# AaltoML/free-hunch

Measured on AMD Instinct MI355X. Metric: images/sec (256x256, num_steps=30, FH-Heun), higher is better.
Workload: dtype f32 UNet (convolutions: exact 3-way bf16 split on the bf16 MFMA, fp32 accuracy) + f64 covariance/CG; 1 GPU; FFHQ-256 arch, gaussian_blur, FH low-rank covariance (dct_diagonal), num_steps=30 heun, batch=8 per GPU; lockstep_groups_per_gpu=2, unet_backend=hip, net_calls_per_image=59

## Files before the change

### free-hunch_amd/csrc/fh_unet.hip

```cpp
#include "fh_common.h"
#include <stdlib.h>

typedef float float16_t __attribute__((ext_vector_type(16)));

namespace {

constexpr int kBK = 32;
constexpr int kLd = kBK + 4;

struct ConvArgs {
  const float* in;
  const float* w;
  const float* bias;
  const float* res;
  float* out;
  int N, H, W, Cin, Cout, KH, KW, pad, stride, Ho, Wo;
  int ksplit;
  float* ws;
};

__device__ __forceinline__ void xcd_tile(int& tile_m, int& tile_n) {
  const unsigned gx = gridDim.x, gy = gridDim.y;
  const unsigned total = gx * gy;
  unsigned lin = blockIdx.y * gx + blockIdx.x;
// ... 740 lines not shown
        if (new_row) load_a(ncc, nky);
      }
      compute(kx, c & 1);
      __syncthreads();
      if (new_row) {
        store_a();
        __syncthreads();
      }
    }
    FH_PHASE(flat_id, 2);
  } else if (!SPLIT || c_begin < c_end) {
  load_a(c_begin / 9, (c_begin / 3) % 3);
  load_b(c_begin / 9, c_begin % 9);
  store_a();
  store_b(0);
  __syncthreads();
  for (int c = c_begin; c < c_end; ++c) {
    const int kx = c % 3;
    const int nx = c + 1;
    const bool more = nx < c_end;
    const bool new_row = more && (nx % 3 == 0);
    if (more) {
      const int ncc = nx / 9, nky = (nx / 3) % 3, nkx = nx % 3;
      load_b(ncc, nky * 3 + nkx);
      if (new_row) load_a(ncc, nky);
    }
    {
      compute(kx, 0);
      __syncthreads();
      if (more) {
        store_b(0);
        if (new_row) store_a();
        __syncthreads();
      }
    }
  }
  }
  const int64_t M = (int64_t)a.N * a.Ho * a.Wo;
  const bool gn = !SPLIT && a.gn_partial != nullptr;
  float* dst = SPLIT ? a.ws + (int64_t)blockIdx.z * M * a.Cout : a.out;
  GnAcc gsum[NI];
#pragma unroll
  for (int j = 0; j < NI; ++j) {
    gsum[j].s0 = gsum[j].s1 = 0.f;
    const int co = n0 + wn + j * 32 + lr;
    if (co >= a.Cout) continue;
    const float bv = (!SPLIT && a.bias != nullptr) ? a.bias[co] : 0.f;
    float tb[5] = {0.f, 0.f, 0.f, 0.f, 0.f};
    if (gn && a.gn_mode == 1) {
#pragma unroll
      for (int q = 0; q < 5; ++q) tb[q] = a.gn_tab[((int64_t)pn * 5 + q) * a.Cout + co];
    }
    if (TT && a.wide) {
      const int k = lane & 3;
      const bool has_res = a.res != nullptr, has_x = gn && a.gn_mode == 1;
#pragma unroll
      for (int i = 0; i < MI; ++i) {
        float4 rw[4], xw[4];
        const int64_t off0 = (m0 + wm + i * 32 + 4 * lh + k) * a.Cout + (co - k);
#pragma unroll
        for (int g = 0; g < 4; ++g) {
          const int64_t off = off0 + (int64_t)(8 * g) * a.Cout;
          rw[g] = has_res ? *reinterpret_cast<const float4*>(a.res + off) : make_float4(0.f, 0.f, 0.f, 0.f);
          xw[g] = has_x ? *reinterpret_cast<const float4*>(a.gn_x + off) : make_float4(0.f, 0.f, 0.f, 0.f);
        }
#pragma unroll
        for (int g = 0; g < 4; ++g) {
          float r4[4] = {rw[g].x, rw[g].y, rw[g].z, rw[g].w}, x4[4] = {xw[g].x, xw[g].y, xw[g].z, xw[g].w}, v4[4];
          if (has_res) quad_transpose(r4, k);
          if (has_x) quad_transpose(x4, k);
#pragma unroll
          for (int q = 0; q < 4; ++q) {
            float v = acc[i][j][4 * g + q];
            v += bv;
            if (has_res) v += r4[q];
            v4[q] = v;
            if (gn) gn_accum_x(a, gsum[j], v, x4[q], tb);
          }
          quad_transpose(v4, k);
          *reinterpret_cast<float4*>(dst + off0 + (int64_t)(8 * g) * a.Cout) = make_float4(v4[0], v4[1], v4[2], v4[3]);
        }
      }
      continue;
    }
#pragma unroll
    for (int i = 0; i < MI; ++i) {
#pragma unroll
      for (int r = 0; r < 16; ++r) {
        const int64_t row = m0 + wm + i * 32 + (r & 3) + 8 * (r >> 2) + 4 * lh;
        if (row < M) {
          float v = acc[i][j][r];
          if (F16 && NP == 2) v = v * ssc.inv_in * ssc.winv;
          v += bv;
          if (!SPLIT && a.res != nullptr) v += a.res[row * a.Cout + co];
          dst[row * a.Cout + co] = v;
          if (gn) gn_accum(a, gsum[j], v, row, co, tb);
        }
      }
    }
  }
  if (GL == 1) FH_PHASE(flat_id, 3);
  if (gn) gn_reduce<NI, BM / 64, WN, BN>(a, gsum, gred, pn, (rem / BM) * (int)gridDim.y + tile_n, n0);
  if (GL == 1) FH_PHASE_EXIT(flat_id);
}

constexpr int kWK = 16;
constexpr int kWLd = kWK + 4;

template <int TB>
__global__ __launch_bounds__(512) void k_conv_wino(ConvArgs a) {
  constexpr int BN = 64;
  __shared__ __align__(16) float Ds[2][2][TB + 2][kWLd];
  __shared__ __align__(16) float Us[2][4][BN][kWLd];
  const int tid = threadIdx.x, lane = tid & 63, wave = tid >> 6;
  constexpr int MI = TB / 128;
  const int wm = (wave >> 1) * (32 * MI), wn = (wave & 1) * 32;
  const int lr = lane & 31, lh = lane >> 5;
  const int Wt = a.W / 2;
  const int64_t Mt = (int64_t)a.N * a.H * Wt;
  const int64_t t0 = (int64_t)blockIdx.x * TB;
  const int n0 = blockIdx.y * BN;
  const int cpt = a.Cin / kWK;
  const int nchunks = 3 * cpt;

  constexpr int NI = (TB + 2) * 8 / 512 + 1;
  int it_y[NI], it_slot[NI], it_q[NI];
  int64_t it_base[NI];
  bool it_ok[NI];
#pragma unroll
  for (int e = 0; e < NI; ++e) {
    const int item = tid + 512 * e;
    const bool has = e < NI - 1 || tid < 16;
    const int ps = item >> 2;
    it_q[e] = (item & 3) * 4;
    it_slot[e] = ps;
    const int64_t tg = t0 + (ps >> 1) - 1;
    it_ok[e] = has && tg >= 0 && tg < Mt;
    it_y[e] = 0;
    it_base[e] = 0;
    if (it_ok[e]) {
      const int n = (int)(tg / ((int64_t)a.H * Wt));
      const int rem = (int)(tg % ((int64_t)a.H * Wt));
      it_y[e] = rem / Wt;
      const int x = (rem % Wt) * 2 + (ps & 1);
      it_base[e] = (((int64_t)n * a.H) * a.W + x) * a.Cin + it_q[e];
    }
    if (!has) it_slot[e] = -1;
  }
  const int ub_pos[2] = {tid >> 8, 2 + (tid >> 8)};
  const int ub_co = (tid >> 2) & 63, ub_q = (tid & 3) * 4;
  const bool uvalid = n0 + ub_co < a.Cout;

  float4 rd[NI], ru[2];
  auto load_chunk = [&](int c) {
    const int ky = c / cpt, c0 = (c % cpt) * kWK;
#pragma unroll
    for (int e = 0; e < NI; ++e) {
      const int hy = it_y[e] + ky - 1;
      const bool ok = it_ok[e] && hy >= 0 && hy < a.H;
      rd[e] = ok ? *reinterpret_cast<const float4*>(a.in + it_base[e] + (int64_t)hy * a.W * a.Cin + c0)
                 : make_float4(0.f, 0.f, 0.f, 0.f);
    }
#pragma unroll
    for (int e = 0; e < 2; ++e) {
      const float* up = a.w + (((int64_t)ub_pos[e] * a.Cout + (uvalid ? n0 + ub_co : 0)) * 3 + ky) * a.Cin + c0 + ub_q;
      ru[e] = uvalid ? *reinterpret_cast<const float4*>(up) : make_float4(0.f, 0.f, 0.f, 0.f);
    }
  };
  auto store_chunk = [&](int buf) {
#pragma unroll
    for (int e = 0; e < NI; ++e)
      if (it_slot[e] >= 0) *reinterpret_cast<float4*>(&Ds[buf][it_slot[e] & 1][it_slot[e] >> 1][it_q[e]]) = rd[e];
    *reinterpret_cast<float4*>(&Us[buf][ub_pos[0]][ub_co][ub_q]) = ru[0];
    *reinterpret_cast<float4*>(&Us[buf][ub_pos[1]][ub_co][ub_q]) = ru[1];
  };

  float mfirst[MI], mlast[MI];
#pragma unroll
  for (int i = 0; i < MI; ++i) {
    const int64_t tg = t0 + wm + i * 32 + lr;
    const int xt = (int)(tg % Wt);
    mfirst[i] = xt == 0 ? 0.f : 1.f;
    mlast[i] = xt == Wt - 1 ? 0.f : 1.f;
  }

  float16_t acc[4][MI];
#pragma unroll
  for (int p = 0; p < 4; ++p)
#pragma unroll
    for (int i = 0; i < MI; ++i)
#pragma unroll
      for (int r = 0; r < 16; ++r) acc[p][i][r] = 0.f;

  load_chunk(0);
  store_chunk(0);
  __syncthreads();
  for (int c = 0; c < nchunks; ++c) {
    const int buf = c & 1;
    if (c + 1 < nchunks) load_chunk(c + 1);
#pragma unroll
    for (int g = 0; g < kWK / 8; ++g) {
      const int ko = g * 8 + 4 * lh;
      float4 v[4][MI], bf[4];
#pragma unroll
      for (int p = 0; p < 4; ++p) bf[p] = *reinterpret_cast<const float4*>(&Us[buf][p][wn + lr][ko]);
#pragma unroll
      for (int i = 0; i < MI; ++i) {
        const int sl = wm + i * 32 + lr + 1;
        const float4 d1 = *reinterpret_cast<const float4*>(&Ds[buf][0][sl][ko]);
        const float4 d2 = *reinterpret_cast<const float4*>(&Ds[buf][1][sl][ko]);
        const float4 d0 = *reinterpret_cast<const float4*>(&Ds[buf][1][sl - 1][ko]);
        const float4 d3 = *reinterpret_cast<const float4*>(&Ds[buf][0][sl + 1][ko]);
        const float f0 = mfirst[i], f3 = mlast[i];
        v[0][i] = make_float4(fmaf(d0.x, f0, -d2.x), fmaf(d0.y, f0, -d2.y), fmaf(d0.z, f0, -d2.z), fmaf(d0.w, f0, -d2.w));
        v[1][i] = make_float4(d1.x + d2.x, d1.y + d2.y, d1.z + d2.z, d1.w + d2.w);
        v[2][i] = make_float4(d2.x - d1.x, d2.y - d1.y, d2.z - d1.z, d2.w - d1.w);
        v[3][i] = make_float4(fmaf(-d3.x, f3, d1.x), fmaf(-d3.y, f3, d1.y), fmaf(-d3.z, f3, d1.z), fmaf(-d3.w, f3, d1.w));
      }
#pragma unroll
      for (int s4 = 0; s4 < 4; ++s4) {
#pragma unroll
        for (int p = 0; p < 4; ++p) {
          const float bv = s4 == 0 ? bf[p].x : s4 == 1 ? bf[p].y : s4 == 2 ? bf[p].z : bf[p].w;
#pragma unroll
          for (int i = 0; i < MI; ++i) {
            const float av = s4 == 0 ? v[p][i].x : s4 == 1 ? v[p][i].y : s4 == 2 ? v[p][i].z : v[p][i].w;
            acc[p][i] = __builtin_amdgcn_mfma_f32_32x32x2f32(av, bv, acc[p][i], 0, 0, 0);
          }
        }
      }
    }
    if (c + 1 < nchunks) store_chunk(buf ^ 1);
    __syncthreads();
  }

  const int co = n0 + wn + lr;
  if (co >= a.Cout) return;
  const float bv = a.bias != nullptr ? a.bias[co] : 0.f;
#pragma unroll
  for (int i = 0; i < MI; ++i) {
#pragma unroll
    for (int r = 0; r < 16; ++r) {
      const int64_t t = t0 + wm + i * 32 + (r & 3) + 8 * (r >> 2) + 4 * lh;
      if (t >= Mt) continue;
      const int n = (int)(t / ((int64_t)a.H * Wt));
      const int rem = (int)(t % ((int64_t)a.H * Wt));
      const int64_t pix = ((int64_t)n * a.H + rem / Wt) * a.W + (rem % Wt) * 2;
      float y0 = acc[0][i][r] + acc[1][i][r] + acc[2][i][r] + bv;
      float y1 = acc[1][i][r] - acc[2][i][r] - acc[3][i][r] + bv;
      if (a.res != nullptr) {
        y0 += a.res[pix * a.Cout + co];
        y1 += a.res[(pix + 1) * a.Cout + co];
      }
      a.out[pix * a.Cout + co] = y0;
      a.out[(pix + 1) * a.Cout + co] = y1;
    }
  }
}

template <int NO>
__global__ __launch_bounds__(256) void k_conv_thin(const float* __restrict__ in, const float* __restrict__ w,
                                                   const float* __restrict__ bias, float* __restrict__ out, int H,
                                                   int W, int Cin, int Cout) {
  constexpr int TS = 16, HS = TS + 2, LD = 36;
  __shared__ __align__(16) float xs[HS * HS][LD];
  const int tid = threadIdx.x, tx = tid & 15, ty = tid >> 4;
  const int x0 = blockIdx.x * TS, y0 = blockIdx.y * TS;
  const int64_t img = blockIdx.z;
  const float* src = in + img * H * W * Cin;
  float acc[NO];
#pragma unroll
  for (int o = 0; o < NO; ++o) acc[o] = 0.f;
  for (int c0 = 0; c0 < Cin; c0 += 32) {
    for (int idx = tid; idx < HS * HS * 8; idx += 256) {
      const int pix = idx >> 3, c4 = (idx & 7) * 4;
      const int gy = y0 + pix / HS - 1, gx = x0 + pix % HS - 1;
      float4 v = make_float4(0.f, 0.f, 0.f, 0.f);
      if (gy >= 0 && gy < H && gx >= 0 && gx < W)
        v = *reinterpret_cast<const float4*>(src + ((int64_t)gy * W + gx) * Cin + c0 + c4);
      *reinterpret_cast<float4*>(&xs[pix][c4]) = v;
    }
    __syncthreads();
#pragma unroll
    for (int tap = 0; tap < 9; ++tap) {
      const int p = (ty + tap / 3) * HS + tx + tap % 3;
#pragma unroll
      for (int c4 = 0; c4 < 32; c4 += 4) {
        const float4 v = *reinterpret_cast<const float4*>(&xs[p][c4]);
#pragma unroll
        for (int o = 0; o < NO; ++o) {
          const float* wp = w + ((int64_t)(o < Cout ? o : 0) * 9 + tap) * Cin + c0 + c4;
          acc[o] = fmaf(v.x, wp[0], fmaf(v.y, wp[1], fmaf(v.z, wp[2], fmaf(v.w, wp[3], acc[o]))));
        }
      }
    }
    __syncthreads();
  }
  const int oy = y0 + ty, ox = x0 + tx;
  if (oy >= H || ox >= W) return;
  float* dst = out + ((img * H + oy) * W + ox) * Cout;
#pragma unroll
  for (int o = 0; o < NO; ++o)
    if (o < Cout) dst[o] = acc[o] + (bias != nullptr ? bias[o] : 0.f);
}

__global__ __launch_bounds__(256) void k_absmax(const float* __restrict__ x, int64_t n, unsigned* __restrict__ out) {
  unsigned m = 0u;
  const int64_t n4 = n >> 2, stride = (int64_t)gridDim.x * 256;
  for (int64_t i = (int64_t)blockIdx.x * 256 + threadIdx.x; i < n4; i += stride) {
    const float4 v = reinterpret_cast<const float4*>(x)[i];
    m = max(max(m, __float_as_uint(fabsf(v.x))), max(__float_as_uint(fabsf(v.y)), max(__float_as_uint(fabsf(v.z)), __float_as_uint(fabsf(v.w)))));
  }
  for (int64_t i = (n4 << 2) + (int64_t)blockIdx.x * 256 + threadIdx.x; i < n; i += stride) m = max(m, __float_as_uint(fabsf(x[i])));
#pragma unroll
  for (int o = 32; o > 0; o >>= 1) m = max(m, (unsigned)__shfl_xor((int)m, o, 64));
  __shared__ unsigned sm[4];
  if ((threadIdx.x & 63) == 0) sm[threadIdx.x >> 6] = m;
  __syncthreads();
  if (threadIdx.x == 0) atomicMax(out + (blockIdx.x % FH_AMAX_SLOTS), max(max(sm[0], sm[1]), max(sm[2], sm[3])));
}

__global__ __launch_bounds__(256) void k_splitk_reduce(const float* __restrict__ ws, const float* __restrict__ bias,
                                                       const float* __restrict__ res, float* __restrict__ out,
                                                       int64_t total, int Cout, int ksplit) {
  for (int64_t i = (int64_t)blockIdx.x * 256 + threadIdx.x; i < total; i += (int64_t)gridDim.x * 256) {
    float v = bias != nullptr ? bias[i % Cout] : 0.f;
    for (int z = 0; z < ksplit; ++z) v += ws[(int64_t)z * total + i];
    if (res != nullptr) v += res[i];
    out[i] = v;
  }
}

struct GemmArgs {
  const float* A;
  const float* B;
  float* C;
  int M, N, K, lda, ldb, ldc, inner;
  int64_t sA0, sA1, sB0, sB1, sC0, sC1;
  float alpha;
};

template <int TA, int TB>
__global__ __launch_bounds__(256) void k_bgemm(GemmArgs g) {
  constexpr int BM = 64, BN = 64;
  __shared__ __align__(16) float As[BM][kLd];
  __shared__ __align__(16) float Bs[BN][kLd];
  const int b0 = blockIdx.z / g.inner, b1 = blockIdx.z % g.inner;
  const float* A = g.A + b0 * g.sA0 + b1 * g.sA1;
  const float* B = g.B + b0 * g.sB0 + b1 * g.sB1;
  float* C = g.C + b0 * g.sC0 + b1 * g.sC1;
  const int tid = threadIdx.x, lane = tid & 63, wave = tid >> 6;
  const int wm = (wave >> 1) * 32, wn = (wave & 1) * 32, lr = lane & 31, lh = lane >> 5;
  const int m0 = blockIdx.x * BM, n0 = blockIdx.y * BN;
  float16_t acc;
#pragma unroll
  for (int r = 0; r < 16; ++r) acc[r] = 0.f;
  for (int k0 = 0; k0 < g.K; k0 += kBK) {
    if (TA == 0) {
      const int row = tid >> 2, col = (tid & 3) * 8;
#pragma unroll
      for (int e = 0; e < 8; ++e) {
        const int gm = m0 + row, gk = k0 + col + e;
        As[row][col + e] = (gm < g.M && gk < g.K) ? A[(int64_t)gm * g.lda + gk] : 0.f;
      }
    } else {
      const int kk = tid >> 3, col = (tid & 7) * 8;
#pragma unroll
      for (int e = 0; e < 8; ++e) {
        const int gm = m0 + col + e, gk = k0 + kk;
        As[col + e][kk] = (gm < g.M && gk < g.K) ? A[(int64_t)gk * g.lda + gm] : 0.f;
      }
    }
    if (TB == 0) {
      const int row = tid >> 2, col = (tid & 3) * 8;
#pragma unroll
      for (int e = 0; e < 8; ++e) {
        const int gn = n0 + row, gk = k0 + col + e;
        Bs[row][col + e] = (gn < g.N && gk < g.K) ? B[(int64_t)gn * g.ldb + gk] : 0.f;
      }
    } else {
      const int kk = tid >> 3, col = (tid & 7) * 8;
#pragma unroll
      for (int e = 0; e < 8; ++e) {
        const int gn = n0 + col + e, gk = k0 + kk;
        Bs[col + e][kk] = (gn < g.N && gk < g.K) ? B[(int64_t)gk * g.ldb + gn] : 0.f;
      }
    }
    __syncthreads();
#pragma unroll
    for (int gq = 0; gq < kBK / 8; ++gq) {
      const float4 af = *reinterpret_cast<const float4*>(&As[wm + lr][gq * 8 + 4 * lh]);
      const float4 bf = *reinterpret_cast<const float4*>(&Bs[wn + lr][gq * 8 + 4 * lh]);
      acc = __builtin_amdgcn_mfma_f32_32x32x2f32(af.x, bf.x, acc, 0, 0, 0);
      acc = __builtin_amdgcn_mfma_f32_32x32x2f32(af.y, bf.y, acc, 0, 0, 0);
      acc = __builtin_amdgcn_mfma_f32_32x32x2f32(af.z, bf.z, acc, 0, 0, 0);
      acc = __builtin_amdgcn_mfma_f32_32x32x2f32(af.w, bf.w, acc, 0, 0, 0);
    }
    __syncthreads();
  }
  const int col = n0 + wn + lr;
  if (col < g.N) {
#pragma unroll
    for (int r = 0; r < 16; ++r) {
      const int row = m0 + wm + (r & 3) + 8 * (r >> 2) + 4 * lh;
      if (row < g.M) C[(int64_t)row * g.ldc + col] = g.alpha * acc[r];
    }
  }
}

struct GnGrid {
  int chunk, nchunks;
};
static inline GnGrid gn_grid(int N, int P) {
  int c = 512;
  while (c > 32 && (int64_t)N * ((P + c - 1) / c) < 256) c >>= 1;
  return {c, (P + c - 1) / c};
}

template <int MODE>
__global__ __launch_bounds__(256) void k_gn_partial(const float* __restrict__ x, const float* __restrict__ dy,
                                                    const float* __restrict__ stats, const float* __restrict__ gamma,
                                                    const float* __restrict__ beta, const float* __restrict__ scale,
                                                    const float* __restrict__ shift, int ss_stride,
                                                    double* __restrict__ partial, int P, int C, int act, int nchunks,
                                                    int kGnChunk) {
  __shared__ double acc[64];
  const int n = blockIdx.x / nchunks, chunk = blockIdx.x % nchunks;
  const int cg = C / 32, c4n = C / 4;
  if (threadIdx.x < 64) acc[threadIdx.x] = 0.0;
  __syncthreads();
  const int p0 = chunk * kGnChunk;
  const int p1 = p0 + kGnChunk < P ? p0 + kGnChunk : P;
  const int lanes_p = c4n >= 256 ? 1 : 256 / c4n;
  const int active = c4n >= 256 ? 256 : lanes_p * c4n;
  if ((int)threadIdx.x < active) {
    for (int c4 = threadIdx.x % (c4n < 256 ? c4n : 256); c4 < c4n; c4 += 256) {
      const int psub = c4n >= 256 ? 0 : threadIdx.x / c4n;
      double s0[4] = {0, 0, 0, 0}, s1[4] = {0, 0, 0, 0};
      float ga[4], be[4], sc[4], sh[4], mean[4], rstd[4];
      if (MODE == 1) {
#pragma unroll
        for (int e = 0; e < 4; ++e) {
          const int c = 4 * c4 + e;
          ga[e] = gamma[c], be[e] = beta[c];
          sc[e] = scale != nullptr ? 1.f + scale[(int64_t)n * ss_stride + c] : 1.f;
          sh[e] = shift != nullptr ? shift[(int64_t)n * ss_stride + c] : 0.f;
          mean[e] = stats[((int64_t)n * 32 + c / cg) * 2], rstd[e] = stats[((int64_t)n * 32 + c / cg) * 2 + 1];
        }
      }
      for (int pb = p0 + psub; pb < p1; pb += 4 * lanes_p) {
        float4 xv[4], gv[4];
        bool ok[4];
#pragma unroll
        for (int u = 0; u < 4; ++u) {
          const int p = pb + u * lanes_p;
          ok[u] = p < p1;
          const int64_t idx = ((int64_t)n * P + (ok[u] ? p : p0)) * C + 4 * c4;
          xv[u] = *reinterpret_cast<const float4*>(x + idx);
          if (MODE == 1) gv[u] = *reinterpret_cast<const float4*>(dy + idx);
        }
#pragma unroll
        for (int u = 0; u < 4; ++u) {
          if (!ok[u]) continue;
          const float xs[4] = {xv[u].x, xv[u].y, xv[u].z, xv[u].w};
          if (MODE == 0) {
#pragma unroll
            for (int e = 0; e < 4; ++e) {
              s0[e] += xs[e];
              s1[e] += (double)xs[e] * xs[e];
            }
          } else {
            const float gs[4] = {gv[u].x, gv[u].y, gv[u].z, gv[u].w};
#pragma unroll
            for (int e = 0; e < 4; ++e) {
              const float xh = (xs[e] - mean[e]) * rstd[e];
              const float t = (xh * ga[e] + be[e]) * sc[e] + sh[e];
              float g = gs[e];
              if (act) {
                const float sg = 1.f / (1.f + __expf(-t));
                g *= sg * (1.f + t * (1.f - sg));
              }
              g *= sc[e] * ga[e];
              s0[e] += g;
              s1[e] += (double)g * xh;
            }
          }
        }
      }
#pragma unroll
      for (int e = 0; e < 4; ++e) {
        const int grp = (4 * c4 + e) / cg;
        atomicAdd(&acc[2 * grp], s0[e]);
        atomicAdd(&acc[2 * grp + 1], s1[e]);
      }
    }
  }
  __syncthreads();
  if (threadIdx.x < 64) partial[(int64_t)blockIdx.x * 64 + threadIdx.x] = acc[threadIdx.x];
}

template <int MODE>
__global__ __launch_bounds__(1024) void k_gn_finalize(const double* __restrict__ partial, float* __restrict__ out,
                                                      int nchunks, double count) {
  __shared__ double red[16][64];
  const int n = blockIdx.x, slot = threadIdx.x & 63, rg = threadIdx.x >> 6;
  double s0 = 0.0, s1 = 0.0;
  int c = rg;
  for (; c + 16 < nchunks; c += 32) {
    s0 += partial[((int64_t)n * nchunks + c) * 64 + slot];
    s1 += partial[((int64_t)n * nchunks + c + 16) * 64 + slot];
  }
  if (c < nchunks) s0 += partial[((int64_t)n * nchunks + c) * 64 + slot];
  red[rg][slot] = s0 + s1;
  __syncthreads();
  if (threadIdx.x >= 64) return;
  double s = 0.0;
#pragma unroll
  for (int g = 0; g < 16; ++g) s += red[g][slot];
  const int grp = slot >> 1, which = slot & 1;
  const double other = __shfl_xor(s, 1, 64);
  if (MODE == 1) {
    out[((int64_t)n * 32 + grp) * 2 + which] = (float)(s / count);
  } else {
    const double sum = which ? other : s, sq = which ? s : other;
    const double mean = sum / count;
    double var = sq / count - mean * mean;
    var = var < 0 ? 0 : var;
    out[((int64_t)n * 32 + grp) * 2 + which] = which ? (float)(1.0 / sqrt(var + 1e-5)) : (float)mean;
  }
}


typedef float f4v_t __attribute__((ext_vector_type(4)));
__device__ __forceinline__ float4 ld_stream(const float* p, int nt) {
  if (nt) {
    const f4v_t v = __builtin_nontemporal_load(reinterpret_cast<const f4v_t*>(p));
    return make_float4(v.x, v.y, v.z, v.w);
  }
  return *reinterpret_cast<const float4*>(p);
}

template <int BWD, bool AMAX = false>
__global__ __launch_bounds__(256) void k_gn_stream(const float* __restrict__ x, const float* __restrict__ dy,
                                                   const float* __restrict__ stats, const float* __restrict__ sums,
                                                   const float* __restrict__ gamma, const float* __restrict__ beta,
                                                   const float* __restrict__ scale, const float* __restrict__ shift,
                                                   int ss_stride, float* __restrict__ out, int P, int C, int act,
                                                   int accumulate, int nchunks, int kGnChunk,
                                                   const float* __restrict__ acc_src = nullptr,
                                                   const float* __restrict__ add2 = nullptr, float* __restrict__ out2 = nullptr,
                                                   int csplit = 0, unsigned* __restrict__ amax = nullptr, int nt = 0) {
  unsigned mx0 = 0u, mx1 = 0u;
  const int n = blockIdx.x / nchunks, chunk = blockIdx.x % nchunks;
  const int cg = C / 32, c4n = C / 4;
  const int p0 = chunk * kGnChunk;
  const int p1 = p0 + kGnChunk < P ? p0 + kGnChunk : P;
  const int lanes_p = c4n >= 256 ? 1 : 256 / c4n;
  const int active = c4n >= 256 ? 256 : lanes_p * c4n;
  const bool live = (int)threadIdx.x < active;
  if (!live && !(BWD && AMAX)) return;
  for (int c4 = threadIdx.x % (c4n < 256 ? c4n : 256); live && c4 < c4n; c4 += 256) {
    const int psub = c4n >= 256 ? 0 : threadIdx.x / c4n;
    float A[4], Bc[4], mean[4], rstd[4], gsc[4], sa[4], sb[4];
#pragma unroll
    for (int e = 0; e < 4; ++e) {
      const int c = 4 * c4 + e;
      const int64_t si = ((int64_t)n * 32 + c / cg) * 2;
      mean[e] = stats[si], rstd[e] = stats[si + 1];
      const float sc = scale != nullptr ? 1.f + scale[(int64_t)n * ss_stride + c] : 1.f;
      const float sh = shift != nullptr ? shift[(int64_t)n * ss_stride + c] : 0.f;
      const float rg = rstd[e] * gamma[c];
      A[e] = rg * sc;
      Bc[e] = (beta[c] - mean[e] * rg) * sc + sh;
      gsc[e] = sc * gamma[c];
      if (BWD) sa[e] = sums[si], sb[e] = sums[si + 1];
    }
    for (int pb = p0 + psub; pb < p1; pb += 4 * lanes_p) {
      float4 xv[4], gv[4], ov[4];
      bool ok[4];
#pragma unroll
      for (int u = 0; u < 4; ++u) {
        const int p = pb + u * lanes_p;
        ok[u] = p < p1;
        const int64_t idx = ((int64_t)n * P + (ok[u] ? p : p0)) * C + 4 * c4;
        xv[u] = *reinterpret_cast<const float4*>(x + idx);
        if (BWD) {
          gv[u] = ld_stream(dy + idx, nt);
          if (accumulate) ov[u] = ld_stream((acc_src != nullptr ? acc_src : out) + idx, nt);
          if (add2 != nullptr) {
            const float4 t2 = ld_stream(add2 + idx, nt);
            if (accumulate)
              ov[u].x += t2.x, ov[u].y += t2.y, ov[u].z += t2.z, ov[u].w += t2.w;
            else
              ov[u] = t2;
          }
        }
      }
#pragma unroll
      for (int u = 0; u < 4; ++u) {
        if (!ok[u]) continue;
        const int64_t idx = ((int64_t)n * P + pb + u * lanes_p) * C + 4 * c4;
        const float xs[4] = {xv[u].x, xv[u].y, xv[u].z, xv[u].w};
        float o[4];
        if (!BWD) {
#pragma unroll
          for (int e = 0; e < 4; ++e) {
// ... 442 lines not shown
      p.bm = 128, p.segw = 32;
    else
      p.reuse = false, p.bm = 128;
    p.gl = p.bm == 256;
  } else if (ksplit > 1 && Cout > 64 && b128 * ksplit >= 256) {
    p.bm = 128;
    const bool r3 = KH == 3 && KW == 3 && pad == 1 && stride == 1 && ((int64_t)H * W) % 128 == 0 && splitk_reuse_enabled();
    if (r3 && W % 128 == 0)
      p.reuse = p.split = true, p.segw = 128;
    else if (r3 && W == 64 && H % 2 == 0)
      p.reuse = p.split = true, p.segw = 64;
    else if (r3 && W == 32 && H % 4 == 0)
      p.reuse = p.split = true, p.segw = 32;
    else if (r3 && W == 16 && H % 8 == 0)
      p.reuse = p.split = true, p.segw = 16;
  } else if (ksplit == 1 && Cout > 64 && ((M + 63) / 64) * nb128 >= 256) {
    p.bm = 64;
  } else {
    p.bm = 64, p.bn = 64;
  }
  p.grid = dim3((unsigned)((M + p.bm - 1) / p.bm), (unsigned)((Cout + p.bn - 1) / p.bn), (unsigned)ksplit);
  p.block = dim3(p.reuse ? 4 * p.bm : (p.bm == 128 ? 512 : 256));
  p.gn_bm = (ksplit == 1 && Cout > 64 && p.bn == 128 && Cout % 32 == 0 && (Ho * Wo) % p.bm == 0) ? p.bm : 0;
  return p;
}

bool conv_tile_tail_enabled() {
  static const bool on = !(getenv("FH_CONV_TILE_TAIL") != nullptr && atoi(getenv("FH_CONV_TILE_TAIL")) == 0);
  return on;
}

template <int SEGW, bool NORM, int BM, int GL, bool SPLIT = false>
void launch_x6r(const X6Plan& p, hipStream_t st, const ConvArgsX& a) {
  switch (g_conv_np) {
    case 1: hipLaunchKernelGGL((k_conv_x6r<SEGW, NORM, BM, 1, GL, false, SPLIT>), p.grid, p.block, 0, st, a); break;
    case 2: hipLaunchKernelGGL((k_conv_x6r<SEGW, NORM, BM, 2, GL, false, SPLIT>), p.grid, p.block, 0, st, a); break;
    case 16: hipLaunchKernelGGL((k_conv_x6r<SEGW, NORM, BM, 1, GL, true, SPLIT>), p.grid, p.block, 0, st, a); break;
    case 32: hipLaunchKernelGGL((k_conv_x6r<SEGW, NORM, BM, 2, GL == 1 ? 2 : GL, true, SPLIT>), p.grid, p.block, 0, st, a); break;
    default: hipLaunchKernelGGL((k_conv_x6r<SEGW, NORM, BM, 3, GL, false, SPLIT>), p.grid, p.block, 0, st, a); break;
  }
}

template <int MI, int NI, int WM, int WN, int MINW>
void launch_x6(const X6Plan& p, hipStream_t st, const ConvArgsX& a) {
  switch (g_conv_np) {
    case 1: hipLaunchKernelGGL((k_conv_x6<MI, NI, WM, WN, MINW, 1>), p.grid, p.block, 0, st, a); break;
    case 2: hipLaunchKernelGGL((k_conv_x6<MI, NI, WM, WN, MINW, 2>), p.grid, p.block, 0, st, a); break;
    case 16: hipLaunchKernelGGL((k_conv_x6<MI, NI, WM, WN, MINW, 1, true>), p.grid, p.block, 0, st, a); break;
    case 32: hipLaunchKernelGGL((k_conv_x6<MI, NI, WM, WN, MINW, 2, true>), p.grid, p.block, 0, st, a); break;
    default: hipLaunchKernelGGL((k_conv_x6<MI, NI, WM, WN, MINW, 3>), p.grid, p.block, 0, st, a); break;
  }
}

constexpr int tile_key(int bm, int w, int gl = 0) { return (bm * 1024 + w) * 2 + gl; }

template <int SEGW, bool NORM>
void launch_x6r_256(const X6Plan& p, hipStream_t st, const ConvArgsX& a) {
  if (g_conv_np == 3 && conv_tile_tail_enabled())
    hipLaunchKernelGGL((k_conv_x6r<SEGW, NORM, 256, 3, 1, false, false, true>), p.grid, p.block, 0, st, a);
  else
    launch_x6r<SEGW, NORM, 256, 1>(p, st, a);
}

template <bool NORM>
bool launch_x6r_tile(const X6Plan& p, hipStream_t st, const ConvArgsX& a) {
  switch (tile_key(p.bm, p.segw, p.gl)) {
    case tile_key(256, 256, 1): launch_x6r_256<256, NORM>(p, st, a); return true;
    case tile_key(256, 128, 1): launch_x6r_256<128, NORM>(p, st, a); return true;
    case tile_key(256, 64, 1): launch_x6r_256<64, NORM>(p, st, a); return true;
    case tile_key(128, 128, 0): launch_x6r<128, NORM, 128, 0>(p, st, a); return true;
    case tile_key(128, 64, 0): launch_x6r<64, NORM, 128, 0>(p, st, a); return true;
    case tile_key(128, 32, 0): launch_x6r<32, NORM, 128, 0>(p, st, a); return true;
  }
  return false;
}

bool launch_x6r_split_tile(const X6Plan& p, hipStream_t st, const ConvArgsX& a) {
  if (p.norm || p.bm != 128 || p.gl != 0) return false;
  switch (p.segw) {
    case 128: launch_x6r<128, false, 128, 0, true>(p, st, a); return true;
    case 64: launch_x6r<64, false, 128, 0, true>(p, st, a); return true;
    case 32: launch_x6r<32, false, 128, 0, true>(p, st, a); return true;
    case 16: launch_x6r<16, false, 128, 0, true>(p, st, a); return true;
  }
  return false;
}

bool launch_x6_tile(const X6Plan& p, hipStream_t st, const ConvArgsX& a) {
  switch (tile_key(p.bm, p.bn)) {
    case tile_key(128, 128): launch_x6<2, 1, 2, 4, 4>(p, st, a); return true;
    case tile_key(64, 128): launch_x6<1, 2, 2, 2, 2>(p, st, a); return true;
    case tile_key(64, 64): launch_x6<1, 1, 2, 2, 2>(p, st, a); return true;
  }
  return false;
}

}

extern "C" {

int fh_unet_set_precision(int mode) {
  if (mode < 0 || mode > 4) return FH_EINVAL;
  g_conv_np = mode == 0 ? 3 : (mode == 1 ? 1 : (mode == 2 ? 2 : (mode == 3 ? 16 : 32)));
  return 0;
}

int fh_unet_get_precision(void) {
  return g_conv_np == 3 ? 0 : (g_conv_np == 1 ? 1 : (g_conv_np == 2 ? 2 : (g_conv_np == 16 ? 3 : 4)));
}

int fh_absmax_f32(const float* x, int64_t n, float* out, void* stream) {
  if (!out || n < 0 || (n > 0 && !x) || ((uintptr_t)x & 15)) return FH_EINVAL;
  hipStream_t st = (hipStream_t)stream;
  FH_CHECK(hipMemsetAsync(out, 0, FH_AMAX_SLOTS * sizeof(float), st));
  if (n > 0) {
    const int64_t want = (n / 4 + 255) / 256;
    hipLaunchKernelGGL(k_absmax, dim3((unsigned)(want < 1 ? 1 : (want > 2048 ? 2048 : want))), dim3(256), 0, st, x, n,
                       reinterpret_cast<unsigned*>(out));
  }
  FH_LAUNCH_CHECK();
  return 0;
}

int fh_conv2d_splitk(int N, int Ho, int Wo, int Cin, int Cout, int KH, int KW) {
  const int64_t M = (int64_t)N * Ho * Wo;
  const int64_t blocks = ((M + 63) / 64) * ((Cout + 63) / 64);
  const int nchunks = KH * KW * (Cin / kBK);
  int z = 1;
  constexpr int target = 2048;
  constexpr int zmax = 8;
  while (blocks * z < target && z < zmax && nchunks / (2 * z) >= 6) z *= 2;
  return z;
}

int fh_conv2d_nhwc(const float* in, const float* w, const float* bias, const float* res, float* out, float* ws,
                   int ksplit, int N, int H, int W, int Cin, int Cout, int KH, int KW, int pad, int stride,
                   void* stream) {
  if (!in || !w || !out || N < 1 || H < 1 || W < 1 || Cin < kBK || Cin % kBK != 0 || Cout < 1 || stride < 1)
    return FH_EINVAL;
  if (ksplit < 1 || ksplit > 32 || (ksplit > 1 && !ws)) return FH_EINVAL;
  ConvArgs a;
  a.in = in, a.w = w, a.bias = bias, a.res = res, a.out = out;
  a.N = N, a.H = H, a.W = W, a.Cin = Cin, a.Cout = Cout, a.KH = KH, a.KW = KW, a.pad = pad, a.stride = stride;
  a.Ho = (H + 2 * pad - KH) / stride + 1;
  a.Wo = (W + 2 * pad - KW) / stride + 1;
  a.ksplit = ksplit, a.ws = ws;
  const int64_t M = (int64_t)N * a.Ho * a.Wo;
  hipStream_t st = (hipStream_t)stream;
  const unsigned Z = (unsigned)ksplit;
  const int64_t b128 = ((M + 127) / 128) * ((Cout + 127) / 128);
  if (ksplit == 1 && Cout > 64 && b128 >= 384) {
    hipLaunchKernelGGL((k_conv_igemm<2, 2>), dim3((unsigned)((M + 127) / 128), (Cout + 127) / 128, 1), dim3(256), 0, st, a);
  } else if (ksplit == 1 && Cout > 64 && ((M + 63) / 64) * ((Cout + 127) / 128) >= 256) {
    hipLaunchKernelGGL((k_conv_igemm<1, 2>), dim3((unsigned)((M + 63) / 64), (Cout + 127) / 128, 1), dim3(256), 0, st, a);
  } else {
    hipLaunchKernelGGL((k_conv_igemm<1, 1>), dim3((unsigned)((M + 63) / 64), (Cout + 63) / 64, Z), dim3(256), 0, st, a);
  }
  if (ksplit > 1) {
    const int64_t total = M * Cout;
    hipLaunchKernelGGL(k_splitk_reduce, dim3(grid_for(total)), dim3(256), 0, st, (const float*)ws, bias, res, out, total,
                       Cout, ksplit);
  }
  FH_LAUNCH_CHECK();
  return 0;
}

int fh_conv2d_x6_gn_chunks(int ksplit, int N, int H, int W, int Cin, int Cout, int KH, int KW, int pad, int stride) {
  if (N < 1 || H < 1 || W < 1 || Cout < 1 || stride < 1) return 0;
  const X6Plan p = x6_plan(ksplit, N, H, W, Cin, Cout, KH, KW, pad, stride, false);
  const int Ho = (H + 2 * pad - KH) / stride + 1, Wo = (W + 2 * pad - KW) / stride + 1;
  return p.gn_bm ? (Ho * Wo / p.gn_bm) * ((Cout + 127) / 128) : 0;
}

int fh_conv2d_x6_plan(int ksplit, int N, int H, int W, int Cin, int Cout, int KH, int KW, int pad, int stride,
                      int32_t* plan) {
  if (!plan || N < 1 || H < 1 || W < 1 || Cin < kBK || Cin % kBK != 0 || Cout < 1 || stride < 1 || ksplit < 1 || ksplit > 32)
    return FH_EINVAL;
  const X6Plan p = x6_plan(ksplit, N, H, W, Cin, Cout, KH, KW, pad, stride, false);
  plan[0] = !p.reuse ? 0 : (p.split ? 2 : 1);
  plan[1] = p.bm, plan[2] = p.bn, plan[3] = p.reuse ? p.segw : 0, plan[4] = p.reuse ? p.gl : 0;
  plan[5] = (int32_t)p.grid.x, plan[6] = (int32_t)p.grid.y, plan[7] = (int32_t)p.grid.z;
  return 0;
}

#ifdef FH_CONV_PHASE_CLOCKS
static unsigned long long* g_phase_buf = nullptr;
int fh_conv_phase_buffer(void* buf) {
  g_phase_buf = (unsigned long long*)buf;
  return 0;
}
#endif

static int set_gn(ConvArgsX& a, const fh_gn_epilogue* epi, int chunks) {
  a.gn_partial = nullptr, a.gn_x = nullptr, a.gn_tab = nullptr, a.gn_mode = a.gn_act = a.gn_chunks = 0;
  a.in_amax = epi != nullptr ? epi->in_amax : nullptr, a.in_scale = 1.f;
  if (g_conv_np == 32 && a.ab == nullptr && a.in_amax == nullptr) return FH_EINVAL;
  if (a.ab != nullptr) a.in_amax = nullptr, a.in_scale = 16.f;
  if (epi == nullptr || epi->partial == nullptr) return 0;
  if (chunks <= 0 || epi->mode < 0 || epi->mode > 1 || (epi->mode == 1 && (!epi->x || !epi->tab))) return FH_EINVAL;
  a.gn_partial = epi->partial, a.gn_x = epi->x, a.gn_tab = epi->tab;
  a.gn_mode = epi->mode, a.gn_act = epi->act, a.gn_chunks = chunks;
  return 0;
}

static int conv2d_x6_launch(const float* in, bool norm, const float* ab_table, int act, const void* wx, const float* bias,
                            const float* res, float* out, float* ws, int ksplit, int N, int H, int W, int Cin, int Cout,
                            int KH, int KW, int pad, int stride, const fh_gn_epilogue* epi, void* stream) {
  if (!in || !wx || !out || N < 1 || H < 1 || W < 1 || Cin < kBK || Cin % kBK != 0 || Cout < 1 || stride < 1)
    return FH_EINVAL;
  if (ksplit < 1 || ksplit > 32 || (ksplit > 1 && !ws)) return FH_EINVAL;
  const X6Plan p = x6_plan(ksplit, N, H, W, Cin, Cout, KH, KW, pad, stride, norm);
  if (norm && (!ab_table || !p.reuse)) return FH_EINVAL;
  ConvArgsX a;
  a.ab = norm ? ab_table : nullptr, a.act = norm ? act : 0;
  a.in = in, a.wx = (const __bf16*)wx, a.bias = bias, a.res = res, a.out = out;
  a.N = N, a.H = H, a.W = W, a.Cin = Cin, a.Cout = Cout, a.KH = KH, a.KW = KW, a.pad = pad, a.stride = stride;
  a.Ho = (H + 2 * pad - KH) / stride + 1;
  a.Wo = (W + 2 * pad - KW) / stride + 1;
  a.ksplit = ksplit, a.ws = ws;
  {
    const int rc = set_gn(a, epi, p.gn_bm ? (a.Ho * a.Wo / p.gn_bm) * ((Cout + 127) / 128) : 0);
    if (rc) return rc;
  }
#ifdef FH_CONV_PHASE_CLOCKS
  a.phase = g_phase_buf;
#endif
  a.wide = Cout % 4 == 0 && (((uintptr_t)out | (uintptr_t)res | (uintptr_t)a.gn_x) & 15) == 0;
  hipStream_t st = (hipStream_t)stream;
  const bool built = !p.reuse ? launch_x6_tile(p, st, a)
                     : p.split ? launch_x6r_split_tile(p, st, a)
                     : p.norm ? launch_x6r_tile<true>(p, st, a)
                              : launch_x6r_tile<false>(p, st, a);
  if (!built) return FH_ESIZE;
  if (ksplit > 1) {
    const int64_t total = (int64_t)N * a.Ho * a.Wo * Cout;
    hipLaunchKernelGGL(k_splitk_reduce, dim3(grid_for(total)), dim3(256), 0, st, (const float*)ws, bias, res, out, total,
                       Cout, ksplit);
  }
  FH_LAUNCH_CHECK();
  return 0;
}

int fh_conv2d_x6_nhwc(const float* in, const void* wx, const float* bias, const float* res, float* out, float* ws,
                      int ksplit, int N, int H, int W, int Cin, int Cout, int KH, int KW, int pad, int stride,
                      void* stream) {
  return conv2d_x6_launch(in, false, nullptr, 0, wx, bias, res, out, ws, ksplit, N, H, W, Cin, Cout, KH, KW, pad, stride,
                          nullptr, stream);
}

int fh_conv2d_x6_nhwc_gn(const float* in, const void* wx, const float* bias, const float* res, float* out, float* ws,
                         int ksplit, int N, int H, int W, int Cin, int Cout, int KH, int KW, int pad, int stride,
                         const fh_gn_epilogue* epi, void* stream) {
  return conv2d_x6_launch(in, false, nullptr, 0, wx, bias, res, out, ws, ksplit, N, H, W, Cin, Cout, KH, KW, pad, stride,
                          epi, stream);
}

__global__ __launch_bounds__(256) void k_gn_table(const float* __restrict__ stats, const float* __restrict__ gamma,
                                                  const float* __restrict__ beta, const float* __restrict__ scale,
                                                  const float* __restrict__ shift, int ss_stride,
                                                  float* __restrict__ table, int C) {
  const int n = blockIdx.x, cg = C / 32;
  for (int c = threadIdx.x; c < C; c += 256) {
    const int64_t si = ((int64_t)n * 32 + c / cg) * 2;
    const float mean = stats[si], rstd = stats[si + 1];
    const float sc = scale != nullptr ? 1.f + scale[(int64_t)n * ss_stride + c] : 1.f;
    const float sh = shift != nullptr ? shift[(int64_t)n * ss_stride + c] : 0.f;
    const float rg = rstd * gamma[c];
    table[((int64_t)n * 2 + 0) * C + c] = rg * sc;
    table[((int64_t)n * 2 + 1) * C + c] = (beta[c] - mean * rg) * sc + sh;
  }
}

int fh_groupnorm_table(const float* stats, const float* gamma, const float* beta, const float* scale, const float* shift,
                       int ss_stride, float* table, int N, int C, void* stream) {
  if (!stats || !gamma || !beta || !table || N < 1 || C % 32 != 0) return FH_EINVAL;
  hipLaunchKernelGGL(k_gn_table, dim3(N), dim3(256), 0, (hipStream_t)stream, stats, gamma, beta, scale, shift, ss_stride,
                     table, C);
  FH_LAUNCH_CHECK();
  return 0;
}

int fh_conv2d_x6_norm_supported(int N, int H, int W, int Cin, int Cout) {
  if (N < 1 || H < 1 || W < 1 || Cin < kBK || Cin % kBK != 0 || Cout < 1) return 0;
  return x6_plan(1, N, H, W, Cin, Cout, 3, 3, 1, 1, true).reuse;
}

int fh_conv2d_x6_norm_nhwc(const float* in, const float* ab_table, int act, const void* wx, const float* bias,
                           const float* res, float* out, int N, int H, int W, int Cin, int Cout, void* stream) {
  return conv2d_x6_launch(in, true, ab_table, act, wx, bias, res, out, nullptr, 1, N, H, W, Cin, Cout, 3, 3, 1, 1, nullptr,
                          stream);
}

int fh_conv2d_x6_norm_nhwc_gn(const float* in, const float* ab_table, int act, const void* wx, const float* bias,
                              const float* res, float* out, int N, int H, int W, int Cin, int Cout, const fh_gn_epilogue* epi,
                              void* stream) {
  return conv2d_x6_launch(in, true, ab_table, act, wx, bias, res, out, nullptr, 1, N, H, W, Cin, Cout, 3, 3, 1, 1, epi,
                          stream);
}

int fh_conv3x3_thin_nhwc(const float* in, const float* w, const float* bias, float* out, int N, int H, int W, int Cin,
                         int Cout, void* stream) {
  if (!in || !w || !out || N < 1 || N > 65535 || H < 1 || W < 1 || Cin < 32 || Cin % 32 != 0 || Cout < 1 || Cout > 8)
    return FH_EINVAL;
  const dim3 grid((W + 15) / 16, (H + 15) / 16, N);
  if (Cout <= 4)
    hipLaunchKernelGGL(k_conv_thin<4>, grid, dim3(256), 0, (hipStream_t)stream, in, w, bias, out, H, W, Cin, Cout);
  else
    hipLaunchKernelGGL(k_conv_thin<8>, grid, dim3(256), 0, (hipStream_t)stream, in, w, bias, out, H, W, Cin, Cout);
  FH_LAUNCH_CHECK();
  return 0;
}

int fh_conv3x3_wino_nhwc(const float* in, const float* wu, const float* bias, const float* res, float* out, int N,
                         int H, int W, int Cin, int Cout, void* stream) {
  if (!in || !wu || !out || N < 1 || H < 1 || W < 2 || (W & 1) || Cin < kWK || Cin % kWK != 0 || Cout < 1)
    return FH_EINVAL;
  ConvArgs a;
  a.in = in, a.w = wu, a.bias = bias, a.res = res, a.out = out;
  a.N = N, a.H = H, a.W = W, a.Cin = Cin, a.Cout = Cout, a.KH = 3, a.KW = 3, a.pad = 1, a.stride = 1;
  a.Ho = H, a.Wo = W, a.ksplit = 1, a.ws = nullptr;
  const int64_t Mt = (int64_t)N * H * (W / 2);
  const int nb = (Cout + 63) / 64;
  if (((Mt + 255) / 256) * nb >= 224)
    hipLaunchKernelGGL(k_conv_wino<256>, dim3((unsigned)((Mt + 255) / 256), nb, 1), dim3(512), 0, (hipStream_t)stream, a);
  else
    hipLaunchKernelGGL(k_conv_wino<128>, dim3((unsigned)((Mt + 127) / 128), nb, 1), dim3(512), 0, (hipStream_t)stream, a);
  FH_LAUNCH_CHECK();
  return 0;
}

int fh_bgemm_f32(const float* A, const float* B, float* C, int M, int N, int K, int lda, int ldb, int ldc, int transA,
                 int transB, int batch, int inner, int64_t sA0, int64_t sA1, int64_t sB0, int64_t sB1, int64_t sC0,
                 int64_t sC1, float alpha, void* stream) {
  if (!A || !B || !C || M < 1 || N < 1 || K < 1 || batch < 1 || inner < 1) return FH_EINVAL;
  GemmArgs g;
  g.A = A, g.B = B, g.C = C, g.M = M, g.N = N, g.K = K, g.lda = lda, g.ldb = ldb, g.ldc = ldc, g.inner = inner;
  g.sA0 = sA0, g.sA1 = sA1, g.sB0 = sB0, g.sB1 = sB1, g.sC0 = sC0, g.sC1 = sC1, g.alpha = alpha;
  dim3 grid((M + 63) / 64, (N + 63) / 64, batch);
  hipStream_t st = (hipStream_t)stream;
  if (!transA && !transB) hipLaunchKernelGGL((k_bgemm<0, 0>), grid, dim3(256), 0, st, g);
  else if (!transA && transB) hipLaunchKernelGGL((k_bgemm<0, 1>), grid, dim3(256), 0, st, g);
  else if (transA && !transB) hipLaunchKernelGGL((k_bgemm<1, 0>), grid, dim3(256), 0, st, g);
  else hipLaunchKernelGGL((k_bgemm<1, 1>), grid, dim3(256), 0, st, g);
  FH_LAUNCH_CHECK();
  return 0;
}

int64_t fh_groupnorm_scratch_doubles(int N, int P) { return (int64_t)N * gn_grid(N, P).nchunks * 64; }

int fh_groupnorm_stats(const float* x, float* stats, double* scratch, int N, int P, int C, void* stream) {
  if (!x || !stats || !scratch || C % 32 != 0) return FH_EINVAL;
  gn_launch_sums<0>((hipStream_t)stream, x, nullptr, nullptr, nullptr, nullptr, nullptr, nullptr, 0, scratch, stats, N, P, C, 0);
  FH_LAUNCH_CHECK();
  return 0;
}

int fh_groupnorm_apply(const float* x, const float* stats, const float* gamma, const float* beta, const float* scale,
                       const float* shift, int ss_stride, float* y, int N, int P, int C, int act, void* stream) {
  if (!x || !stats || !gamma || !beta || !y || C % 32 != 0) return FH_EINVAL;
  const GnGrid g = gn_grid(N, P);
  hipLaunchKernelGGL(k_gn_stream<0>, dim3(N * g.nchunks), dim3(256), 0, (hipStream_t)stream, x, (const float*)nullptr,
                     stats, (const float*)nullptr, gamma, beta, scale, shift, ss_stride, y, P, C, act, 0, g.nchunks, g.chunk);
  FH_LAUNCH_CHECK();
  return 0;
}

int fh_groupnorm_bwd(const float* x, const float* dy, const float* stats, const float* gamma, const float* beta,
                     const float* scale, const float* shift, int ss_stride, float* sums, double* scratch, float* dx, int N,
                     int P, int C, int act, int accumulate, void* stream) {
  if (!x || !dy || !stats || !gamma || !beta || !sums || !scratch || !dx || C % 32 != 0) return FH_EINVAL;
  hipStream_t st = (hipStream_t)stream;
  gn_launch_sums<1>(st, x, dy, stats, gamma, beta, scale, shift, ss_stride, scratch, sums, N, P, C, act);
  gn_launch_bwd_stream(st, x, dy, stats, sums, gamma, beta, scale, shift, ss_stride, accumulate ? dx : nullptr, nullptr, dx,
                       nullptr, 0, N, P, C, act, nullptr);
  FH_LAUNCH_CHECK();
  return 0;
}

int fh_groupnorm_finalize(const double* partial, float* out, int N, int chunks, double count, int mode, void* stream) {
  if (!partial || !out || N < 1 || chunks < 1 || count <= 0 || mode < 0 || mode > 1) return FH_EINVAL;
  if (mode == 0)
    hipLaunchKernelGGL(k_gn_finalize<0>, dim3(N), dim3(1024), 0, (hipStream_t)stream, partial, out, chunks, count);
  else
    hipLaunchKernelGGL(k_gn_finalize<1>, dim3(N), dim3(1024), 0, (hipStream_t)stream, partial, out, chunks, count);
  FH_LAUNCH_CHECK();
  return 0;
}

__global__ __launch_bounds__(256) void k_gn_bwd_table(const float* __restrict__ stats, const float* __restrict__ gamma,
                                                      const float* __restrict__ beta, const float* __restrict__ scale,
                                                      const float* __restrict__ shift, int ss_stride,
                                                      float* __restrict__ table, int C) {
  const int n = blockIdx.x, cg = C / 32;
  for (int c = threadIdx.x; c < C; c += 256) {
    const int64_t si = ((int64_t)n * 32 + c / cg) * 2;
    const float mean = stats[si], rstd = stats[si + 1];
    const float sc = scale != nullptr ? 1.f + scale[(int64_t)n * ss_stride + c] : 1.f;
    const float sh = shift != nullptr ? shift[(int64_t)n * ss_stride + c] : 0.f;
    const float rg = rstd * gamma[c];
    float* t = table + (int64_t)n * 5 * C + c;
    t[0] = rg * sc;
    t[C] = (beta[c] - mean * rg) * sc + sh;
    t[2 * C] = mean;
    t[3 * C] = rstd;
    t[4 * C] = sc * gamma[c];
  }
}

int fh_groupnorm_bwd_table(const float* stats, const float* gamma, const float* beta, const float* scale, const float* shift,
                           int ss_stride, float* table, int N, int C, void* stream) {
  if (!stats || !gamma || !beta || !table || N < 1 || C % 32 != 0) return FH_EINVAL;
  hipLaunchKernelGGL(k_gn_bwd_table, dim3(N), dim3(256), 0, (hipStream_t)stream, stats, gamma, beta, scale, shift, ss_stride,
                     table, C);
  FH_LAUNCH_CHECK();
  return 0;
}

int fh_groupnorm_bwd_apply(const float* x, const float* dy, const float* stats, const float* sums, const float* gamma,
                           const float* beta, const float* scale, const float* shift, int ss_stride, float* dx, int N, int P,
                           int C, int act, int accumulate, void* stream) {
  return fh_groupnorm_bwd_apply_ex(x, dy, stats, sums, gamma, beta, scale, shift, ss_stride, accumulate ? dx : nullptr, nullptr,
                                   dx, nullptr, 0, N, P, C, act, nullptr, stream);
}

int fh_groupnorm_bwd_sums(const float* x, const float* dy, const float* stats, const float* gamma, const float* beta,
                          const float* scale, const float* shift, int ss_stride, float* sums, double* scratch, int N, int P,
                          int C, int act, void* stream) {
  if (!x || !dy || !stats || !gamma || !beta || !sums || !scratch || C % 32 != 0) return FH_EINVAL;
  gn_launch_sums<1>((hipStream_t)stream, x, dy, stats, gamma, beta, scale, shift, ss_stride, scratch, sums, N, P, C, act);
  FH_LAUNCH_CHECK();
  return 0;
}

int fh_groupnorm_bwd_apply_ex(const float* x, const float* dy, const float* stats, const float* sums, const float* gamma,
                              const float* beta, const float* scale, const float* shift, int ss_stride, const float* acc_src,
                              const float* add2, float* dx, float* dx2, int csplit, int N, int P, int C, int act, float* amax2,
                              void* stream) {
  if (!x || !dy || !stats || !sums || !gamma || !beta || !dx || C % 32 != 0) return FH_EINVAL;
  if (dx2 != nullptr && (csplit <= 0 || csplit >= C || csplit % 4 != 0)) return FH_EINVAL;
  gn_launch_bwd_stream((hipStream_t)stream, x, dy, stats, sums, gamma, beta, scale, shift, ss_stride, acc_src, add2, dx, dx2,
                       csplit, N, P, C, act, amax2);
  FH_LAUNCH_CHECK();
  return 0;
}

int fh_groupnorm_small_supported(int P, int C) {
  static const int max_pixels = getenv("FH_GN_SMALL_MAX_PIXELS") ? atoi(getenv("FH_GN_SMALL_MAX_PIXELS")) : kGnSmallMaxPixels;
  if (P < 1 || P > max_pixels || C < 32 || C % 32 != 0 || (C / 32) % 4 != 0 || C / 128 > kGnSmallThreads) return 0;
  const int lanes = kGnSmallThreads / (C / 128);
  return (int64_t)P * (C / 32) <= kGnSmallLimit && (P + lanes - 1) / lanes <= kGnSmallMaxIpt ? 1 : 0;
}

int fh_groupnorm_fwd_small(const float* x, const float* gamma, const float* beta, const float* scale, const float* shift,
                           int ss_stride, float* y, float* stats, int N, int P, int C, int act, void* stream) {
  if (!fh_groupnorm_small_supported(P, C) || !x || !gamma || !beta || !y || !stats || N < 1) return FH_EINVAL;
  gn_small_dispatch<GnSmallFwd>(P, C, (hipStream_t)stream, N, x, gamma, beta, scale, shift, ss_stride, y, stats, P, C, act);
  FH_LAUNCH_CHECK();
  return 0;
}

int fh_groupnorm_bwd_small(const float* x, const float* dy, const float* stats, float* sums, const float* gamma,
                           const float* beta, const float* scale, const float* shift, int ss_stride, const float* acc_src,
                           const float* add2, float* dx, float* dx2, int csplit, int N, int P, int C, int act, void* stream) {
  if (!fh_groupnorm_small_supported(P, C) || !x || !dy || !stats || !gamma || !beta || !dx || N < 1) return FH_EINVAL;
  if (dx2 != nullptr && (csplit <= 0 || csplit >= C || csplit % 4 != 0)) return FH_EINVAL;
  gn_small_dispatch<GnSmallBwd>(P, C, (hipStream_t)stream, N, x, dy, stats, sums, gamma, beta, scale, shift, ss_stride, acc_src,
                                add2, dx, dx2, csplit, P, C, act);
  FH_LAUNCH_CHECK();
  return 0;
}

int fh_softmax_rows(float* s, int64_t rows, int T, void* stream) {
  if (!s || rows < 1 || T < 1) return FH_EINVAL;
  hipLaunchKernelGGL(k_softmax_rows, dim3((unsigned)rows), dim3(256), 0, (hipStream_t)stream, s, T);
  FH_LAUNCH_CHECK();
  return 0;
}

int fh_softmax_bwd_rows(const float* p, float* dp, int64_t rows, int T, void* stream) {
  if (!p || !dp || rows < 1 || T < 1) return FH_EINVAL;
  hipLaunchKernelGGL(k_softmax_bwd_rows, dim3((unsigned)rows), dim3(256), 0, (hipStream_t)stream, p, dp, T);
  FH_LAUNCH_CHECK();
  return 0;
}

int fh_resample2x(const float* in, float* out, int N, int Hs, int Ws, int C, int mode, void* stream) {
  if (!in || !out || C % 4 != 0 || mode < 0 || mode > 4) return FH_EINVAL;
  const int64_t items = (int64_t)N * Hs * Ws * (C / 4) * ((mode == 0 || mode == 3) ? 1 : 4);
  hipLaunchKernelGGL(k_resample, dim3(grid_for(items)), dim3(256), 0, (hipStream_t)stream, in, out, N, Hs, Ws, C, mode);
  FH_LAUNCH_CHECK();
  return 0;
}

int fh_concat_channels(float* a, float* b, float* out, int64_t P, int Ca, int Cb, int split, void* stream) {
  if (!a || !b || !out || Ca % 4 != 0 || Cb % 4 != 0) return FH_EINVAL;
  hipLaunchKernelGGL(k_concat, dim3(grid_for(P * ((Ca + Cb) / 4))), dim3(256), 0, (hipStream_t)stream, a, b, out, P, Ca,
                     Cb, split);
  FH_LAUNCH_CHECK();
  return 0;
}

int fh_layout_nchw_nhwc(const float* in, float* out, int N, int C, int64_t P, int Cp, int to_nhwc, void* stream) {
  if (!in || !out || Cp < C) return FH_EINVAL;
  if (to_nhwc)
    hipLaunchKernelGGL(k_nchw_to_nhwc, dim3(grid_for((int64_t)N * P * Cp)), dim3(256), 0, (hipStream_t)stream, in, out, N,
                       C, P, Cp);
  else
    hipLaunchKernelGGL(k_nhwc_to_nchw, dim3(grid_for((int64_t)N * P * C)), dim3(256), 0, (hipStream_t)stream, in, out, N,
                       C, P, Cp);
  FH_LAUNCH_CHECK();
  return 0;
}

int fh_add_f32(const float* a, const float* b, float* out, int64_t n, void* stream) {
  if (!a || !b || !out || n % 4 != 0) return FH_EINVAL;
  hipLaunchKernelGGL(k_add_f32, dim3(grid_for(n / 4)), dim3(256), 0, (hipStream_t)stream, a, b, out, n / 4);
  FH_LAUNCH_CHECK();
  return 0;
}

}
```

Measured before the change: 2.577 images/s.

## Add strip-tiled thin-output 3x3 conv kernel with register prefetch and swizzled LDS

```diff
diff --git a/free-hunch_amd/csrc/fh_unet.hip b/free-hunch_amd/csrc/fh_unet.hip
--- a/free-hunch_amd/csrc/fh_unet.hip
+++ b/free-hunch_amd/csrc/fh_unet.hip
@@ -1066,6 +1066,142 @@
 #pragma unroll
   for (int o = 0; o < NO; ++o)
     if (o < Cout) dst[o] = acc[o] + (bias != nullptr ? bias[o] : 0.f);
+}
+
+constexpr int kThinTile = 32, kThinHalo = kThinTile + 2, kThinPitch = kThinHalo + 1;
+constexpr int kThinPixQuads = kThinHalo * kThinPitch * 8;
+constexpr unsigned kThinNoPix = 0xffffffffu;
+constexpr int kThinLoads = (kThinHalo * kThinHalo * 8 + 255) / 256;
+
+template <int NO>
+__global__ __launch_bounds__(256) void k_conv_thin_strip(const float* __restrict__ in, const float* __restrict__ w,
+                                                         const float* __restrict__ bias, float* __restrict__ out, int H,
+                                                         int W, int Cin, int Cout) {
+  extern __shared__ __align__(16) float thin_lds[];
+  float4* xs = reinterpret_cast<float4*>(thin_lds);
+  float* wsf = thin_lds + kThinPixQuads * 4;
+  const float4* ws = reinterpret_cast<const float4*>(wsf);
+  const int tid = threadIdx.x, sx = tid & 7, ty = tid >> 3;
+  const int x0 = blockIdx.x * kThinTile, y0 = blockIdx.y * kThinTile;
+  const int64_t img = blockIdx.z;
+  const float* src = in + img * H * W * Cin;
+  float acc[4][NO];
+#pragma unroll
+  for (int j = 0; j < 4; ++j)
+#pragma unroll
+    for (int o = 0; o < NO; ++o) acc[j][o] = 0.f;
+  unsigned gpix[kThinLoads];
+  const int q4 = (tid & 7) * 4;
+  float4 pf[kThinLoads];
+#pragma unroll
+  for (int u = 0; u < kThinLoads; ++u) {
+    const int idx = tid + u * 256, pix = idx >> 3, q = idx & 7;
+    const int row = pix / kThinHalo, col = pix - row * kThinHalo;
+    const int gy = y0 + row - 1, gx = x0 + col - 1;
+    const bool inside = idx < kThinHalo * kThinHalo * 8 && gy >= 0 && gy < H && gx >= 0 && gx < W;
+    gpix[u] = inside ? (unsigned)gy * (unsigned)W + (unsigned)gx : kThinNoPix;
+    pf[u] = make_float4(0.f, 0.f, 0.f, 0.f);
+    if (inside) pf[u] = *reinterpret_cast<const float4*>(src + (int64_t)gpix[u] * Cin + q4);
+  }
+  constexpr int kWLoads = (NO * 288 + 255) / 256;
+  float wpf[kWLoads];
+#pragma unroll
+  for (int u = 0; u < kWLoads; ++u) {
+    const int idx = tid + u * 256, o = idx / 288, rem = idx - o * 288;
+    wpf[u] = idx < NO * 288 ? w[(int64_t)((o < Cout ? o : 0) * 9 + (rem >> 5)) * Cin + (rem & 31)] : 0.f;
+  }
+  for (int c0 = 0; c0 < Cin; c0 += 32) {
+#pragma unroll
+    for (int u = 0; u < kThinLoads; ++u) {
+      const int idx = tid + u * 256, pix = idx >> 3, q = idx & 7;
+      const int row = pix / kThinHalo, col = pix - row * kThinHalo;
+      if (idx < kThinHalo * kThinHalo * 8)
+        xs[(row * kThinPitch + col) * 8 + (q ^ (((col >> 2) & 3) | (((row >> 1) & 1) << 2)))] = pf[u];
+    }
+    if (c0 + 32 < Cin) {
+#pragma unroll
+      for (int u = 0; u < kThinLoads; ++u)
+        if (gpix[u] != kThinNoPix) pf[u] = *reinterpret_cast<const float4*>(src + (int64_t)gpix[u] * Cin + q4 + c0 + 32);
+    }
+#pragma unroll
+    for (int u = 0; u < kWLoads; ++u) {
+      const int idx = tid + u * 256, o = idx / 288, rem = idx - o * 288, tap = rem >> 5, c = rem & 31;
+      if (idx < NO * 288) wsf[(((tap * 8 + (c >> 2)) * NO + o) << 2) + (c & 3)] = wpf[u];
+      if (c0 + 32 < Cin && idx < NO * 288) wpf[u] = w[(int64_t)((o < Cout ? o : 0) * 9 + tap) * Cin + c0 + 32 + c];
+    }
+    __syncthreads();
+#pragma unroll 1
+    for (int tap = 0; tap < 9; ++tap) {
+      const int ky = tap / 3, kx = tap - 3 * ky, row = ty + ky;
+      const float4* wt = ws + tap * 8 * NO;
+      int pb[4], sw[4];
+#pragma unroll
+      for (int j = 0; j < 4; ++j) {
+        const int col = 4 * sx + j + kx;
+        pb[j] = (row * kThinPitch + col) * 8;
+        sw[j] = ((col >> 2) & 3) | (((row >> 1) & 1) << 2);
+      }
+      constexpr int kSets = NO < 8 ? 2 : 1;
+      float4 wv[kSets][NO], vv[kSets][4];
+      if (kSets == 2) {
+#pragma unroll
+        for (int o = 0; o < NO; ++o) wv[0][o] = wt[o];
+#pragma unroll
+        for (int j = 0; j < 4; ++j) vv[0][j] = xs[pb[j] + sw[j]];
+      }
+#pragma unroll
+      for (int q = 0; q < 8; ++q) {
+        const int qn = q + kSets - 1, sn = qn & (kSets - 1);
+        if (qn < 8) {
+#pragma unroll
+          for (int o = 0; o < NO; ++o) wv[sn][o] = wt[qn * NO + o];
+#pragma unroll
+          for (int j = 0; j < 4; ++j) vv[sn][j] = xs[pb[j] + (qn ^ sw[j])];
+        }
+        if (kSets == 2) __builtin_amdgcn_sched_barrier(0);
+#pragma unroll
+        for (int j = 0; j < 4; ++j) {
+          const float4 v = vv[q & (kSets - 1)][j];
+#pragma unroll
+          for (int o = 0; o < NO; ++o) {
+            const float4 wq = wv[q & (kSets - 1)][o];
+            acc[j][o] = fmaf(v.x, wq.x, fmaf(v.y, wq.y, fmaf(v.z, wq.z, fmaf(v.w, wq.w, acc[j][o]))));
+          }
+        }
+        if (kSets == 2) __builtin_amdgcn_sched_barrier(0);
+      }
+    }
+    __syncthreads();
+  }
+  const int oy = y0 + ty;
+  if (oy >= H) return;
+#pragma unroll
+  for (int j = 0; j < 4; ++j) {
+    const int ox = x0 + 4 * sx + j;
+    if (ox >= W) continue;
+    float* dst = out + ((img * H + oy) * W + ox) * Cout;
+#pragma unroll
+    for (int o = 0; o < NO; ++o)
+      if (o < Cout) dst[o] = acc[j][o] + (bias != nullptr ? bias[o] : 0.f);
+  }
+}
+
+static bool conv_thin_strip_on() {
+  static const bool on = !(getenv("FH_CONV_THIN") != nullptr && atoi(getenv("FH_CONV_THIN")) == 0);
+  return on;
+}
+
+template <int NO>
+static int conv_thin_strip_launch(const float* in, const float* w, const float* bias, float* out, int N, int H, int W, int Cin,
+                                  int Cout, hipStream_t st) {
+  constexpr int lds = (kThinPixQuads + 72 * NO) * 16;
+  static const hipError_t opt_in =
+      hipFuncSetAttribute((const void*)k_conv_thin_strip<NO>, hipFuncAttributeMaxDynamicSharedMemorySize, lds);
+  if (opt_in != hipSuccess) return (int)opt_in;
+  const dim3 grid((W + kThinTile - 1) / kThinTile, (H + kThinTile - 1) / kThinTile, N);
+  hipLaunchKernelGGL(k_conv_thin_strip<NO>, grid, dim3(256), lds, st, in, w, bias, out, H, W, Cin, Cout);
+  FH_LAUNCH_CHECK();
+  return 0;
 }
 
 __global__ __launch_bounds__(256) void k_absmax(const float* __restrict__ x, int64_t n, unsigned* __restrict__ out) {
@@ -2114,6 +2250,12 @@
                          int Cout, void* stream) {
   if (!in || !w || !out || N < 1 || N > 65535 || H < 1 || W < 1 || Cin < 32 || Cin % 32 != 0 || Cout < 1 || Cout > 8)
     return FH_EINVAL;
+  if (conv_thin_strip_on()) {
+    if (Cout <= 3) return conv_thin_strip_launch<3>(in, w, bias, out, N, H, W, Cin, Cout, (hipStream_t)stream);
+    if (Cout == 4) return conv_thin_strip_launch<4>(in, w, bias, out, N, H, W, Cin, Cout, (hipStream_t)stream);
+    if (Cout <= 6) return conv_thin_strip_launch<6>(in, w, bias, out, N, H, W, Cin, Cout, (hipStream_t)stream);
+    return conv_thin_strip_launch<8>(in, w, bias, out, N, H, W, Cin, Cout, (hipStream_t)stream);
+  }
   const dim3 grid((W + 15) / 16, (H + 15) / 16, N);
   if (Cout <= 4)
     hipLaunchKernelGGL(k_conv_thin<4>, grid, dim3(256), 0, (hipStream_t)stream, in, w, bias, out, H, W, Cin, Cout);
```

Result: no change. 2.583 images/s (median of 4 runs) (+0.2%).
